# TimeEscaper/distributed_eigenspaces

Hardware: AMD Instinct MI355X
Metric: samples/sec ingested + time-to-eigenspace (d=8192,k=64) at 1/8 GPU; sinθ error (higher is better)
Workload: dtype f32

## Files before the change

__graft_entry__.py:

```python
import os
import sys

ROOT = os.path.dirname(os.path.abspath(__file__))
if ROOT not in sys.path:
    sys.path.insert(0, ROOT)


def build() -> None:
    from distributed_eigenspaces_amd import _build
    _build.build_library(force=True)
    _build.build_oja_timeout_lib()
    import distributed_eigenspaces_amd
    from distributed_eigenspaces_amd import _lib
    _lib.lib()


def smoke() -> None:
    import numpy as np
    import torch

    import distributed_eigenspaces_amd as de
    from oracle import ref_cpu

    dev = torch.device("cuda", 0)
    rng = np.random.default_rng(0)
    d, k, m, n_i = 256, 8, 4, 1024
    U, _ = np.linalg.qr(rng.standard_normal((d, k)))
    X = rng.standard_normal((m * n_i, d)) + (rng.standard_normal((m * n_i, k)) * 2.0) @ U.T
    X = X.astype(np.float32)
    xs = torch.from_numpy(X).to(dev)
    bases = []
    for i in range(m):
        S = de.sigma_hat(xs[i * n_i:(i + 1) * n_i])
        bases.append(de.topk_eigh(S, k).V)
    res = de.projavg_topk(de.stack_bases(bases), k, 1.0 / m, q0=bases[0])
    torch.cuda.synchronize()
    _, _, sw, sv = ref_cpu.one_shot(X.astype(np.float64), k, m)
    dist = ref_cpu.projector_distance(res.V.cpu().numpy(), sv)
    ev_err = np.max(np.abs(res.evals.cpu().numpy() - sw) / np.abs(sw))
    assert dist <= 1e-4, f"smoke: ||P - P_ref||_F = {dist:.3e}"
    assert ev_err <= 1e-5, f"smoke: eigenvalue rel err {ev_err:.3e}"
    print(f"smoke ok: ||P-P_ref||_F={dist:.2e} eig_rel={ev_err:.2e}")


if __name__ == "__main__":
    cmd = sys.argv[1] if len(sys.argv) > 1 else "build"
    {"build": build, "smoke": smoke}[cmd]()
```

distributed_eigenspaces_amd/_build.py:

```python
from __future__ import annotations

import os
import shutil
import subprocess
import sys

HERE = os.path.dirname(os.path.abspath(__file__))
CSRC = os.path.join(HERE, "csrc")
LIB = os.path.join(HERE, "libdeig.so")
SOURCES = ["capi.hip", "syrk.hip", "syrk_split.hip", "syrk_u8.hip", "skinny.hip", "rr.hip", "oja.hip",
           "project.hip", "sweep.hip", "shift.hip"]
EXTRA_FLAGS = {"sweep.hip": ["-fno-slp-vectorize"], "syrk_split.hip": ["-fno-slp-vectorize"]}
HEADERS = ["deig_internal.hpp", os.path.join("..", "..", "include", "deig.h")]
OJA_TIMEOUT_LIB = os.path.join(HERE, "libdeig_test_oja_timeout.so")
ARCH = os.environ.get("DEIG_OFFLOAD_ARCH", "gfx950")


def _hipcc() -> str:
    for cand in (os.environ.get("HIPCC"), "/opt/rocm/bin/hipcc", shutil.which("hipcc")):
        if cand and os.path.exists(cand):
            return cand
    raise RuntimeError("hipcc not found (ROCm required to build libdeig.so)")


def _stale() -> bool:
    if not os.path.exists(LIB):
        return True
    t = os.path.getmtime(LIB)
    deps = [os.path.join(CSRC, s) for s in SOURCES + HEADERS]
    return any(os.path.getmtime(p) > t for p in deps)


def build_library(force: bool = False, verbose: bool = True, defines=(), out: str | None = None) -> str:
    lib = out or LIB
    if not force and not defines and lib == LIB and not _stale():
        return LIB
    objs = []
    tmpdir = os.path.join(HERE, "build" if not defines else "build_ab")
    os.makedirs(tmpdir, exist_ok=True)
    hipcc = _hipcc()
    procs = []
    for src in SOURCES:
        obj = os.path.join(tmpdir, src.replace(".hip", ".o"))
        objs.append(obj)
        cmd = [hipcc, f"--offload-arch={ARCH}", "-O3", "-std=c++17", "-fPIC", "-Wall",
               "-Wno-unused-function", "-Wno-inline-asm"] + list(defines) + EXTRA_FLAGS.get(src, []) + \
            ["-c", os.path.join(CSRC, src), "-o", obj]
        procs.append((cmd, subprocess.Popen(cmd, stdout=subprocess.PIPE, stderr=subprocess.STDOUT)))
    for cmd, p in procs:
        out, _ = p.communicate()
        if p.returncode != 0:
            raise RuntimeError("hipcc failed:\n" + " ".join(cmd) + "\n" + out.decode())
        if verbose and out.strip():
            sys.stderr.write(out.decode())
    tmp_lib = lib + ".tmp"
    cmd = [hipcc, f"--offload-arch={ARCH}", "-shared", "-fPIC", "-o", tmp_lib] + objs
    r = subprocess.run(cmd, stdout=subprocess.PIPE, stderr=subprocess.STDOUT)
    if r.returncode != 0:
        raise RuntimeError("link failed:\n" + r.stdout.decode())
    os.replace(tmp_lib, lib)
    if verbose:
        sys.stderr.write(f"built {lib}\n")
    return lib


def build_oja_timeout_lib(verbose: bool = True) -> str:
    tmpdir = os.path.join(HERE, "build")
    hipcc = _hipcc()
    obj = os.path.join(tmpdir, "oja_timeout.o")
    cmd = [hipcc, f"--offload-arch={ARCH}", "-O3", "-std=c++17", "-fPIC", "-Wall", "-Wno-unused-function",
           "-Wno-inline-asm", "-DDEIG_AB_OJA_SPIN_TICKS=0", "-c", os.path.join(CSRC, "oja.hip"), "-o", obj]
    r = subprocess.run(cmd, stdout=subprocess.PIPE, stderr=subprocess.STDOUT)
    if r.returncode != 0:
        raise RuntimeError("hipcc failed:\n" + " ".join(cmd) + "\n" + r.stdout.decode())
    objs = [obj if s == "oja.hip" else os.path.join(tmpdir, s.replace(".hip", ".o")) for s in SOURCES]
    tmp_lib = OJA_TIMEOUT_LIB + ".tmp"
    r = subprocess.run([hipcc, f"--offload-arch={ARCH}", "-shared", "-fPIC", "-o", tmp_lib] + objs,
                       stdout=subprocess.PIPE, stderr=subprocess.STDOUT)
    if r.returncode != 0:
        raise RuntimeError("link failed:\n" + r.stdout.decode())
    os.replace(tmp_lib, OJA_TIMEOUT_LIB)
    if verbose:
        sys.stderr.write(f"built {OJA_TIMEOUT_LIB}\n")
    return OJA_TIMEOUT_LIB


if __name__ == "__main__":
    build_library(force="--force" in sys.argv)
```

distributed_eigenspaces_amd/csrc/syrk_split.hip:

```cpp
#include <cmath>
#include <cstdlib>

#include "deig_internal.hpp"

namespace deig {
namespace {

typedef __bf16 bf16x8 __attribute__((ext_vector_type(8)));
typedef int i32x4 __attribute__((ext_vector_type(4)));
typedef unsigned u32x4 __attribute__((ext_vector_type(4)));
typedef __bf16 bf16x2 __attribute__((ext_vector_type(2)));
typedef float f32x2 __attribute__((ext_vector_type(2)));

__device__ __forceinline__ uint32_t cvt2(float a, float b) {
  return __builtin_bit_cast(uint32_t, __builtin_convertvector(f32x2{a, b}, bf16x2));
}
__device__ __forceinline__ float lo_f(uint32_t p) { return __uint_as_float(p << 16); }
__device__ __forceinline__ float hi_f(uint32_t p) { return __uint_as_float(p & 0xffff0000u); }

constexpr int BT = 256;
constexpr int ROWS_PAD = 32;
constexpr int NTHR = 512;
constexpr int SLICE_B = BT * 16;
constexpr int SLAB = BT * BT;
constexpr int SPLIT_YB = 256;
constexpr int SUPER_H = 8, SUPER_W = 4;
constexpr int BLOCK_B = 8 * SLICE_B;
constexpr size_t DEFAULT_CHUNK_BYTES = size_t(64) << 30;

struct SSched {
  const unsigned char* XP;
  float* S;
  float* part;
  float* accs;
  const int* order;
  int64_t lds, dp;
  int64_t NK;
  int nseg;
  int d, nt, T, G, q, R;
  float alpha;
  int beta;
  int flush_kt;
  int prio;
  unsigned* pace;
  int pace_kt;
  int xm;
  int rpace;
  const float* X;
  int64_t ldx, nrows;
  float* corr;
};

constexpr int kChipPaceEvery = 2;
#ifdef DEIG_AB_SYRK_FLUSH_STAGGER
constexpr int kFlushStaggerDiv = DEIG_AB_SYRK_FLUSH_STAGGER;
#else
constexpr int kFlushStaggerDiv = 16;
#endif

__device__ __noinline__ void xcd_pace(unsigned* ctr, unsigned target) {
  __hip_atomic_fetch_add(ctr, 1u, __ATOMIC_RELAXED, __HIP_MEMORY_SCOPE_AGENT);
  const uint64_t t0 = wall_clock64();
  while (__hip_atomic_load(ctr, __ATOMIC_RELAXED, __HIP_MEMORY_SCOPE_AGENT) < target) {
    if (wall_clock64() - t0 > 2000) break;
    __builtin_amdgcn_s_sleep(1);
  }
}


__device__ __forceinline__ i32x4 make_rsrc(const void* base, uint32_t nrec) {
  const uint64_t a = reinterpret_cast<uint64_t>(base);
  i32x4 r;
  r[0] = (int)(uint32_t)a;
  r[1] = (int)((uint32_t)(a >> 32) & 0xffffu);
  r[2] = (int)nrec;
  r[3] = 0x00020000;
  return r;
}

__device__ __forceinline__ void dma16(i32x4 rsrc, int voff, const void* lds_dst) {
  const unsigned m0v = (unsigned)(uintptr_t)(lds_void*)lds_dst;
  asm volatile("s_mov_b32 m0, %2\n\tbuffer_load_dwordx4 %0, %1, 0 offen lds"
               :
               : "v"(voff), "s"(rsrc), "s"(m0v)
               : "memory", "m0");
}

template <int KT>
struct Geo {
  static constexpr int NSLICE = 4 * KT;
  static constexpr int PANEL_B = NSLICE * SLICE_B;
  static constexpr int BUF_B = 2 * PANEL_B;
  static constexpr int DMA = 4 * KT, DMA_DIAG = 2 * KT;
};

template <int KT>
__device__ __forceinline__ void stage(const SSched& s, int64_t kt, int i0, int j0, bool diag,
                                      unsigned char* buf, int wave, int lane16) {
  using G_ = Geo<KT>;
  const int64_t blk = kt * KT / 2;
  const int s0 = (int)((kt * KT) & 1) * 4;
  const i32x4 rsrc = make_rsrc(s.XP + blk * (int64_t)s.nt * BLOCK_B, (uint32_t)(s.nt * BLOCK_B));
  int l16 = lane16;
  asm volatile("" : "+v"(l16));
  if (!diag) {
#pragma unroll
    for (int u = 0; u < KT; ++u) {
      const int c = wave * KT + u;
      const int pb = c / G_::NSLICE, sl = c % G_::NSLICE;
      const int g = (pb ? j0 : i0) / BT * BLOCK_B + (s0 + sl) * SLICE_B;
      unsigned char* dst = buf + pb * G_::PANEL_B + sl * SLICE_B;
#pragma unroll
      for (int p = 0; p < 4; ++p) dma16(rsrc, l16 + g + p * 1024, dst + p * 1024);
    }
  } else {
#pragma unroll
    for (int u = 0; u < 2 * KT; ++u) {
      const int idx = wave * 2 * KT + u;
      const int sl = idx >> 2, p = idx & 3;
      dma16(rsrc, l16 + i0 / BT * BLOCK_B + (s0 + sl) * SLICE_B + p * 1024,
            buf + sl * SLICE_B + p * 1024);
    }
  }
}

constexpr int OCT_B = 2 * SLICE_B;

__device__ __forceinline__ void stage_x(const SSched& s, int64_t kt, int f0, unsigned char* buf,
                                        int wave, int voff) {
  const int64_t row0 = kt * 32 + 8 * (wave & 3);
  int64_t rv = s.nrows - row0;
  rv = rv < 0 ? 0 : rv > 8 ? 8 : rv;
  const uint32_t ldx4 = (uint32_t)s.ldx * 4u;
  const i32x4 rsrc = make_rsrc(s.X + row0 * s.ldx + f0, (uint32_t)rv * ldx4);
  unsigned char* dst = buf + (wave >> 2) * Geo<2>::PANEL_B + (wave & 3) * OCT_B;
#pragma unroll
  for (int r = 0; r < 8; ++r) dma16(rsrc, voff + (int)(r * ldx4), dst + r * 1024);
}

template <bool SQ>
__device__ __forceinline__ void convert_x(unsigned char* buf, int wave, int lane, int rv, int fv,
                                          float* sq) {
  unsigned char* R = buf + (wave >> 2) * Geo<2>::PANEL_B + (wave & 3) * OCT_B;
  f32x2 v[2][8];
#pragma unroll
  for (int h = 0; h < 2; ++h)
#pragma unroll
    for (int r = 0; r < 8; ++r)
      v[h][r] = *reinterpret_cast<const f32x2*>(R + r * 1024 + h * 512 + 8 * lane);
  if (rv < 8 || fv < 256) {
#pragma unroll
// ... 334 lines not shown
          stage<KT>(s, k0 + t + NST - 1, i0, j0, diag, lds + nxt * BUF_B, wave, lane16);
        unsigned char* bc = lds + cur * BUF_B;
        acc.template mma<KT>(bc, diag ? bc : bc + Geo<KT>::PANEL_B, wi, wj, lane);
      }
      if (++since == s.flush_kt && t + 1 < nkt) {
        flush<MF>(slab, !flushed, acc, wave, lane);
        wait_vm<0>();
        flushed = true;
        since = 0;
      }
      cur = cur + 1 == NST ? 0 : cur + 1;
      nxt = nxt + 1 == NST ? 0 : nxt + 1;
    }
  }
  if (flushed) unflush<MF>(slab, acc, wave, lane);
  if (sqw) {
    float* c = s.corr + (int64_t)(cseg * 4 + wave) * s.dp + i0;
#pragma unroll
    for (int h = 0; h < 2; ++h)
      *reinterpret_cast<f32x2*>(c + 128 * h + 2 * lane) = f32x2{sq[2 * h], sq[2 * h + 1]};
  }

  if (partial) {
#pragma unroll
    for (int q = 0; q < NQUAD; ++q)
      *slab_at(slab, wave, q, lane) = f32x4{acc.at(q, 0), acc.at(q, 1), acc.at(q, 2), acc.at(q, 3)};
    return;
  }
#pragma unroll
  for (int q = 0; q < NQUAD; ++q) {
    const float a[4] = {acc.at(q, 0), acc.at(q, 1), acc.at(q, 2), acc.at(q, 3)};
    store4(s, i0 + 128 * wi + Acc<MF>::qrow(q, lane), j0 + 64 * wj + Acc<MF>::qcol(q, lane), diag, a);
  }
}

#ifdef DEIG_AB_SYRK_VARIANT
#include "ab/syrk_split_superseded.inc"
#endif

struct PaceSeq {
  int n;
  unsigned base, mult;
  unsigned gbase = 0;
  unsigned gmult = 0;
  bool g = false;
};

__device__ __forceinline__ int rem_active(const SSched& s, int L, int u) {
  if (s.xm) {
    const int gx = s.G >> 3, left = s.R * s.xm - u * gx;
    return left < 0 ? 0 : (left < gx ? left : gx);
  }
  const int xcd = blockIdx.x & 7;
  const int nx = (s.G >> 3) + (xcd < (s.G & 7) ? 1 : 0);
  const int left = s.R * s.nseg - u * s.G - (L - (int)(blockIdx.x >> 3));
  return left < 0 ? 0 : (left < nx ? left : nx);
}

__device__ __forceinline__ int rem_rounds(const SSched& s, int L) {
  if (s.xm) {
    const int gx = s.G >> 3, l = L % gx, items = s.R * s.xm;
    return l < items ? (items - 1 - l) / gx + 1 : 0;
  }
  const int items = s.R * s.nseg;
  return L < items ? (items - 1 - L) / s.G + 1 : 0;
}

__device__ __forceinline__ void rem_item(const SSched& s, int L, int u, int& tile, int& slot, int& sg) {
  int r;
  if (s.xm) {
    const int gx = s.G >> 3, x = L / gx, j = L - x * gx + u * gx;
    const int sl = j / s.R;
    r = j - sl * s.R;
    sg = x * s.xm + sl;
  } else {
    const int i = L + u * s.G;
    sg = i / s.R;
    r = i - sg * s.R;
  }
  tile = s.q * s.G + r;
  slot = sg * s.R + r;
}

constexpr int kDwOff = -1, kDwDiag = -2;
constexpr bool dw_skip(int dw, int mb, int nb) { return dw >= 0 && 16 * mb + 15 < dw + 16 * nb; }
constexpr bool dw_row(int dw, int mb) { return !dw_skip(dw, mb, 0); }
constexpr bool dw_col(int dw, int nb) { return !dw_skip(dw, 7, nb); }
constexpr bool dw_idle(int dw) { return !dw_row(dw, 7); }

template <int PRIO, int DW>
__device__ __forceinline__ void segment_h(const SSched& s, unsigned char* lds, int tile, int64_t k0,
                                          int64_t k1, int slot, bool partial, const PaceSeq& pc) {
  constexpr bool idle = dw_idle(DW);
#ifndef DEIG_AB_SYRK_DIAG_B_DMA
  constexpr bool dgb = DW != kDwOff;
#else
  constexpr bool dgb = false;
#endif
  constexpr int BUF_B = Geo<2>::BUF_B;
  constexpr int QB = 8 * 1024;
  constexpr int BOFF = 4 * QB;
  const int lane = threadIdx.x & 63;
  const int wave = __builtin_amdgcn_readfirstlane(threadIdx.x >> 6);
  const int wi = wave >> 2, wj = wave & 3;
  const bool lag = wave >= 4;
  const int tt = __builtin_amdgcn_readfirstlane(s.order[tile]);
  const int ti = tt & 0xffff, tj = tt >> 16;
  const int i0 = ti * BT, j0 = tj * BT;
  const bool diag = (ti == tj);
  Acc<16> acc;
  acc.zero();
  float* slab = partial ? s.part + (int64_t)slot * SLAB : s.accs + (int64_t)blockIdx.x * SLAB;
  bool flushed = false;
  const int64_t nkt = k1 - k0;
  auto bar = [&]() {
    __builtin_amdgcn_sched_barrier(0);
    __builtin_amdgcn_s_barrier();
    __builtin_amdgcn_sched_barrier(0);
    asm volatile("" ::: "memory");
  };
  const int a_off = ti * BLOCK_B + wave * SLICE_B + ((lane >> 5) * 128 + (lane & 31)) * 16;
  const int b_off = tj * BLOCK_B + wave * SLICE_B + lane * 16;
  const uint32_t nrec = (uint32_t)(s.nt * BLOCK_B);
  auto ring_rsrc = [&](int64_t kt) {
    return make_rsrc(s.XP + kt * (int64_t)s.nt * BLOCK_B, nrec);
  };
  auto issue_a = [&](int64_t kt, int q, unsigned char* buf) {
    const i32x4 r = ring_rsrc(kt);
    int o = a_off + q * 512;
    asm volatile("" : "+v"(o));
    dma16(r, o, buf + q * QB + wave * 1024);
  };
  auto issue_b = [&](int64_t kt, unsigned char* buf, int p0, int p1) {
    const i32x4 r = ring_rsrc(kt);
    int o = b_off;
    asm volatile("" : "+v"(o));
#pragma unroll
    for (int p = 0; p < 4; ++p)
      if (p >= p0 && p < p1) dma16(r, o + p * 1024, buf + BOFF + wave * SLICE_B + p * 1024);
  };
  if (nkt > 0) {
    wait_vm<0>();
    __syncthreads();
    if constexpr (!dgb) issue_b(k0, lds, 0, 4);
#pragma unroll
    for (int q = 0; q < 4; ++q) issue_a(k0, q, lds);
    if (nkt > 1) {
      if constexpr (!dgb) issue_b(k0 + 1, lds + BUF_B, 0, 2);
      issue_a(k0 + 1, 0, lds + BUF_B);
      issue_a(k0 + 1, 1, lds + BUF_B);
      wait_vm<dgb ? 2 : 4>();
    } else {
      wait_vm<0>();
    }
    asm volatile("s_waitcnt lgkmcnt(0)" ::: "memory");
    bar();
    if (lag) bar();
    const int c = lane & 15, g4 = lane >> 4;
    const int xcd = blockIdx.x & 7;
    int since = kFlushStaggerDiv > 0 ? xcd * (s.flush_kt / kFlushStaggerDiv) : 0;
    int since_pace = 0, pace_left = pc.n;
    unsigned pace_t = pc.base;
    int gcount = 0;
    unsigned gtarget = pc.gbase;
    bf16x8 bhi[4], blo[4];
    bf16x8 ahi[4], alo[4];
    for (int64_t t = 0; t < nkt; ++t) {
      unsigned char* cur = lds + (t & 1) * BUF_B;
      unsigned char* nxt = lds + ((t + 1) & 1) * BUF_B;
      const bool has1 = t + 1 < nkt, has2 = t + 2 < nkt;
      const unsigned char* pa = cur + ((g4 * 2) * 64 + 32 * wi + c) * 16;
      const unsigned char* pb = cur + BOFF + ((g4 * 2) * BT + 64 * wj + c) * 16;
      const unsigned char* pbd = cur + (2 * (wj & 1)) * QB + (2 * g4) * 1024 + (32 * (wj >> 1) + c) * 16;
#pragma unroll
      for (int h = 0; h < 2; ++h) {
        if (h == 0) {
          if (pace_left > 0 && ++since_pace == s.pace_kt) {
            since_pace = 0;
            --pace_left;
            pace_t += pc.mult;
            if (threadIdx.x == 0) xcd_pace(s.pace + 32 * xcd, pace_t);
            if (pc.g && ++gcount == kChipPaceEvery) {
              gcount = 0;
              gtarget += pc.gmult;
              if (threadIdx.x == 0) xcd_pace(s.pace + 32 * 8, gtarget);
            }
          }
          if (since == s.flush_kt) {
            if constexpr (!idle) flush<16>(slab, !flushed, acc, wave, lane);
            wait_vm<0>();
            flushed = true;
            since = 0;
          }
          ++since;
          if (has1) {
            if constexpr (!dgb) issue_b(k0 + t + 1, nxt, 2, 4);
            issue_a(k0 + t + 1, 2, nxt);
            issue_a(k0 + t + 1, 3, nxt);
          }
#pragma unroll
          for (int nb = 0; nb < 4; ++nb) {
            if (dw_col(DW, nb)) {
              if constexpr (dgb) {
                const unsigned char* pq = pbd + (nb >> 1) * QB + (16 * (nb & 1)) * 16;
                bhi[nb] = *reinterpret_cast<const bf16x8*>(pq);
                blo[nb] = *reinterpret_cast<const bf16x8*>(pq + 1024);
              } else {
                bhi[nb] = *reinterpret_cast<const bf16x8*>(pb + (16 * nb) * 16);
                blo[nb] = *reinterpret_cast<const bf16x8*>(pb + (BT + 16 * nb) * 16);
              }
            }
          }
        } else if (has2) {
          if constexpr (!dgb) issue_b(k0 + t + 2, cur, 0, 2);
          issue_a(k0 + t + 2, 0, cur);
          issue_a(k0 + t + 2, 1, cur);
        }
#pragma unroll
        for (int m = 0; m < 4; ++m) {
          const int q = 2 * h + (m >> 1), mm = m & 1;
          if (dw_row(DW, 4 * h + m)) {
            ahi[m] = *reinterpret_cast<const bf16x8*>(pa + q * QB + (16 * mm) * 16);
            alo[m] = *reinterpret_cast<const bf16x8*>(pa + q * QB + (64 + 16 * mm) * 16);
          }
        }
        if constexpr (dgb) {
          if (h == 0) {
            if (has1) wait_vm<4>(); else wait_vm<0>();
          } else {
            if (has2) wait_vm<2>(); else wait_vm<0>();
          }
        } else if (h == 0) {
          if (has1) wait_vm<8>(); else wait_vm<0>();
        } else {
          if (has2) wait_vm<6>(); else if (has1) wait_vm<2>(); else wait_vm<0>();
        }
        asm volatile("s_waitcnt lgkmcnt(0)" ::: "memory");
        bar();
        if (PRIO) __builtin_amdgcn_s_setprio(1);
#pragma unroll
        for (int m = 0; m < 4; ++m) {
          const int mb = 4 * h + m;
#pragma unroll
          for (int nb = 0; nb < 4; ++nb)
            if (!dw_skip(DW, mb, nb))
              acc.a[mb][nb] = __builtin_amdgcn_mfma_f32_16x16x32_bf16(ahi[m], bhi[nb], acc.a[mb][nb], 0, 0, 0);
#pragma unroll
          for (int nb = 0; nb < 4; ++nb)
            if (!dw_skip(DW, mb, nb))
              acc.a[mb][nb] = __builtin_amdgcn_mfma_f32_16x16x32_bf16(ahi[m], blo[nb], acc.a[mb][nb], 0, 0, 0);
#pragma unroll
          for (int nb = 0; nb < 4; ++nb)
            if (!dw_skip(DW, mb, nb))
              acc.a[mb][nb] = __builtin_amdgcn_mfma_f32_16x16x32_bf16(alo[m], bhi[nb], acc.a[mb][nb], 0, 0, 0);
        }
        if (PRIO) __builtin_amdgcn_s_setprio(0);
        bar();
      }
    }
    if (!lag) bar();
  }
  if (flushed && !idle) unflush<16>(slab, acc, wave, lane);
  if (partial) {
#pragma unroll
    for (int q = 0; q < NQUAD; ++q)
      *slab_at(slab, wave, q, lane) = f32x4{acc.at(q, 0), acc.at(q, 1), acc.at(q, 2), acc.at(q, 3)};
    return;
  }
  if constexpr (idle) return;
#pragma unroll
  for (int q = 0; q < NQUAD; ++q) {
    const float a[4] = {acc.at(q, 0), acc.at(q, 1), acc.at(q, 2), acc.at(q, 3)};
    store4(s, i0 + 128 * wi + Acc<16>::qrow(q, lane), j0 + 64 * wj + Acc<16>::qcol(q, lane), diag, a);
  }
}

template <int PRIO>
__global__ __launch_bounds__(NTHR) void syrks_h_kernel(SSched s) {
  __shared__ __attribute__((aligned(16))) unsigned char lds[2 * Geo<2>::BUF_B];
  const int L = xcd_logical(blockIdx.x, s.G);
  const int nwork = s.q + rem_rounds(s, L);
  const int xcd = blockIdx.x & 7;
  const unsigned nx = (unsigned)((s.G >> 3) + (xcd < (s.G & 7) ? 1 : 0));
  const unsigned P = s.pace_kt > 0 ? (unsigned)(s.NK / s.pace_kt) : 0u;
  const int Pm = (s.pace_kt > 0 && s.rpace && s.nseg > 0) ? (int)(s.NK / s.nseg / s.pace_kt) : 0;
  unsigned rbase = (unsigned)s.q * P * nx;
  for (int w = 0; w < nwork; ++w) {
    int tile, slot = 0, sg = 0;
    int64_t k0 = 0, k1 = s.NK;
    const bool partial = w >= s.q;
    PaceSeq pc{0, 0u, 0u};
    if (!partial) {
      tile = w * s.G + L;
      pc = PaceSeq{(int)P, (unsigned)w * P * nx, nx};
      pc.g = true;
      pc.gbase = (unsigned)w * (P / kChipPaceEvery) * (unsigned)s.G;
      pc.gmult = (unsigned)s.G;
    } else {
      rem_item(s, L, w - s.q, tile, slot, sg);
      k0 = __builtin_amdgcn_readfirstlane((int)(s.NK * sg / s.nseg));
      k1 = __builtin_amdgcn_readfirstlane((int)(s.NK * (sg + 1) / s.nseg));
      if (Pm > 0) {
        unsigned before = 0;
        for (int u = 0; u < w - s.q; ++u) before += (unsigned)rem_active(s, L, u);
        pc = PaceSeq{Pm, rbase + before * (unsigned)Pm, (unsigned)rem_active(s, L, w - s.q)};
#ifndef DEIG_AB_SYRK_NO_REM_CHIP
        if (!s.xm) {
          const int items = s.R * s.nseg;
          unsigned gb = (unsigned)s.q * (P / kChipPaceEvery) * (unsigned)s.G;
          for (int u = 0; u < w - s.q; ++u)
            gb += (unsigned)min(s.G, items - u * s.G) * (unsigned)(Pm / kChipPaceEvery);
          pc.g = true;
          pc.gbase = gb;
          pc.gmult = (unsigned)min(s.G, items - (w - s.q) * s.G);
        }
#endif
      }
    }
    const int tt = __builtin_amdgcn_readfirstlane(s.order[tile]);
    const int wv = __builtin_amdgcn_readfirstlane(threadIdx.x >> 6);
    const bool dg = (tt & 0xffff) == (tt >> 16);
#ifndef DEIG_AB_SYRK_NO_DIAG_IDLE
    const int dw = 64 * (wv & 3) - 128 * (wv >> 2);
    if (dg && dw == 0)
      segment_h<PRIO, 0>(s, lds, tile, k0, k1, slot, partial, pc);
    else if (dg && dw == 64)
      segment_h<PRIO, 64>(s, lds, tile, k0, k1, slot, partial, pc);
    else if (dg && dw >= 128)
      segment_h<PRIO, 128>(s, lds, tile, k0, k1, slot, partial, pc);
    else if (dg)
      segment_h<PRIO, kDwDiag>(s, lds, tile, k0, k1, slot, partial, pc);
    else
#endif
      segment_h<PRIO, kDwOff>(s, lds, tile, k0, k1, slot, partial, pc);
  }
}

template <int MF, int KT, int NST, bool FX>
__global__ __launch_bounds__(NTHR) void syrks_kernel(SSched s) {
  static_assert(NST * Geo<KT>::BUF_B <= 160 * 1024, "LDS ring exceeds 160 KiB");
  __shared__ __attribute__((aligned(16))) unsigned char lds[NST * Geo<KT>::BUF_B];
  const int b = blockIdx.x;
  const int L = xcd_logical(b, s.G);
  const int items = s.R * s.nseg;
  const int nwork = s.q + (L < items ? (items - 1 - L) / s.G + 1 : 0);
  for (int w = 0; w < nwork; ++w) {
    int tile, slot = 0, cseg = 0;
    int64_t k0 = 0, k1 = s.NK;
    const bool partial = w >= s.q;
    if (!partial) {
      tile = w * s.G + L;
    } else {
      const int i = L + (w - s.q) * s.G;
      const int sg = i / s.R, r = i - sg * s.R;
      tile = s.q * s.G + r;
      slot = i;
      cseg = sg;
      k0 = __builtin_amdgcn_readfirstlane((int)(s.NK * sg / s.nseg));
      k1 = __builtin_amdgcn_readfirstlane((int)(s.NK * (sg + 1) / s.nseg));
    }
    const int pace_j = (!partial && s.pace_kt > 0) ? (int)(w * (s.NK / s.pace_kt)) : -1;
    if constexpr (FX) {
      const int tt = __builtin_amdgcn_readfirstlane(s.order[tile]);
      if ((tt & 0xffff) == (tt >> 16) && (threadIdx.x >> 6) < 4)
        segment<MF, KT, NST, true, true>(s, lds, tile, k0, k1, slot, partial, pace_j, cseg);
      else
        segment<MF, KT, NST, true, false>(s, lds, tile, k0, k1, slot, partial, pace_j, cseg);
    } else {
      segment<MF, KT, NST, false, false>(s, lds, tile, k0, k1, slot, partial, pace_j, cseg);
    }
  }
}

template <int MF>
__global__ __launch_bounds__(256) void syrks_reduce_kernel(SSched s) {
  const int r = blockIdx.x;
  const int f = blockIdx.y * 256 + threadIdx.x;
  const int lane = f & 63, q = (f >> 6) & (NQUAD - 1), wave = f >> 11;
  const int wi = wave >> 2, wj = wave & 3;
  const int tt = s.order[s.q * s.G + r];
  const int ti = tt & 0xffff, tj = tt >> 16;
  const bool diag = (ti == tj);
  f32x4 sum = {0.f, 0.f, 0.f, 0.f};
  for (int sg = 0; sg < s.nseg; ++sg)
    sum += *reinterpret_cast<const f32x4*>(s.part + (int64_t)(sg * s.R + r) * SLAB + (int64_t)f * 4);
  const float a[4] = {sum[0], sum[1], sum[2], sum[3]};
  store4(s, ti * BT + 128 * wi + Acc<MF>::qrow(q, lane), tj * BT + 64 * wj + Acc<MF>::qcol(q, lane),
         diag, a);
}

__device__ __forceinline__ uint32_t bf16_rne(float x) {
  const uint32_t u = __float_as_uint(x);
  return (u + 0x7fffu + ((u >> 16) & 1u)) >> 16;
}

__global__ __launch_bounds__(256) void split_kernel(const float* __restrict__ X, int64_t n,
                                                    int64_t ldx, int d, int64_t dp, int64_t noct,
// ... 50 lines not shown
  const int i = blockIdx.x * 64 + t;
  float c = 0.f;
  if (i < d) {
#pragma unroll 8
    for (int y = sl; y < yb; y += 4) c += corr[(int64_t)y * dp + i];
  }
  part[sl][t] = c;
  __syncthreads();
  if (sl == 0 && i < d) S[(int64_t)i * lds + i] += alpha * (((part[0][t] + part[1][t]) + part[2][t]) + part[3][t]);
}

__global__ __launch_bounds__(256) void tile_order_kernel(int nt, int* order) {
  const int nsc = (nt + SUPER_W - 1) / SUPER_W;
  const int u = blockIdx.x * 256 + threadIdx.x;
  const int R0 = (u / nsc) * SUPER_H, C0 = (u % nsc) * SUPER_W;
  if (R0 >= nt) return;
  const int rmax = R0 + SUPER_H < nt ? R0 + SUPER_H : nt;
  if (C0 >= rmax) return;
  int idx = R0 * (R0 + 1) / 2;
  for (int c = 0; c < C0; c += SUPER_W)
    for (int ti = R0; ti < rmax; ++ti) {
      const int hi = c + SUPER_W < ti + 1 ? c + SUPER_W : ti + 1;
      idx += hi > c ? hi - c : 0;
    }
  for (int ti = R0; ti < rmax; ++ti)
    for (int tj = C0; tj < C0 + SUPER_W && tj <= ti; ++tj) order[idx++] = ti | (tj << 16);
}

int remainder_segments(int64_t R, int G) {
  if (R <= 0) return 0;
  double best = 1e30;
  for (int k = 1; k <= 64; ++k) best = fmin(best, (double)cdiv(R * k, G) / k);
  for (int k = 1; k <= 64; ++k)
    if ((double)cdiv(R * k, G) / k <= best * 1.02) return k;
  return 1;
}

__global__ __launch_bounds__(256) void tile_order_compact_kernel(int nt, int* order) {
  const int m = nt / 8;
  const int u = blockIdx.x * 256 + threadIdx.x;
  if (u >= m * m) return;
  int a = (int)sqrtf((float)u);
  while (a * a > u) --a;
  while ((a + 1) * (a + 1) <= u) ++a;
  const int item = u - a * a;
  int* grp = order + 32 * u;
  if (item == 0) {
    int i = 0;
    for (int ti = 8 * a; ti < 8 * a + 8; ++ti)
      for (int tj = 8 * a; tj <= ti; ++tj) {
        const int v = ti | (tj << 16);
        if (i < 32) grp[i] = v;
        else order[32 * m * m + 4 * a + (i - 32)] = v;
        ++i;
      }
  } else {
    const int b = (item - 1) >> 1, h = (item - 1) & 1;
    int i = 0;
    for (int ti = 8 * a; ti < 8 * a + 8; ++ti)
      for (int tj = 8 * b + 4 * h; tj < 8 * b + 4 * h + 4; ++tj) grp[i++] = ti | (tj << 16);
  }
}

#ifdef DEIG_AB_SYRK_REM
constexpr int kSyrkRem = DEIG_AB_SYRK_REM;
#else
constexpr int kSyrkRem = 1;
#endif
int syrk_variant(int64_t d);

int xcd_segments(int64_t R, int gx) {
  double best = 1e30;
  for (int k = 1; k <= 8; ++k) best = fmin(best, (double)cdiv(R * k, gx) / (8 * k));
  for (int k = 1; k <= 8; ++k)
    if ((double)cdiv(R * k, gx) / (8 * k) <= best * 1.02) return k;
  return 1;
}

struct Layout {
  int64_t dp, nt, T, G, q, R, nseg, xm, yb_max, chunk_rows;
  size_t off_order, off_pace, off_accs, off_part, off_corr, off_xp, total;
};

Layout make_layout(int64_t n, int64_t d, int G, int64_t chunk_rows) {
  Layout L;
  L.dp = cdiv(d, BT) * BT;
  L.nt = L.dp / BT;
  L.T = L.nt * (L.nt + 1) / 2;
  L.G = G;
  L.q = L.T / G;
  L.R = L.T % G;
  L.nseg = remainder_segments(L.R, G);
  L.xm = 0;
  if ((kSyrkRem & 2) && syrk_variant(d) % 100000 >= 30000 && G % 8 == 0 && L.R > 0) {
    L.xm = xcd_segments(L.R, G / 8);
    L.nseg = 8 * L.xm;
  }
  L.yb_max = SPLIT_YB;
  L.chunk_rows = chunk_rows;
  size_t off = 0;
  L.off_order = off;
  off = align_up(off + sizeof(int) * L.T, 256);
  L.off_pace = off;
  off += 16 * 128;
  L.off_accs = off;
  off += sizeof(float) * (size_t)G * SLAB;
  L.off_part = off;
  off += sizeof(float) * (size_t)(L.R * L.nseg) * SLAB;
  L.off_corr = off;
  off = align_up(off + sizeof(float) * (size_t)L.yb_max * L.dp, 256);
  L.off_xp = off;
  off += (size_t)chunk_rows * L.dp * 4;
  L.total = off;
  (void)n;
  return L;
}

int64_t default_chunk_rows(int64_t n, int64_t d) {
  const int64_t dp = cdiv(d, BT) * BT;
  const int64_t n32 = cdiv(n, ROWS_PAD) * ROWS_PAD;
  int64_t cap = (int64_t)(DEFAULT_CHUNK_BYTES / (size_t)(dp * 4)) / ROWS_PAD * ROWS_PAD;
  if (cap < ROWS_PAD) cap = ROWS_PAD;
  return n32 < cap ? n32 : cap;
}

constexpr int64_t kFusedMaxD = 2048;
#ifdef DEIG_AB_SYRK_VARIANT
constexpr int kSyrkLarge = DEIG_AB_SYRK_VARIANT;
#else
constexpr int kSyrkLarge = 30000;
#endif
int syrk_variant(int64_t d) {
#ifdef DEIG_AB_SYRK_VARIANT
  (void)d;
  return DEIG_AB_SYRK_VARIANT;
#else
  return d <= kFusedMaxD ? 163 : kSyrkLarge;
#endif
}

template <int V>
void launch_split_pass_kernel(int G, hipStream_t stream, const SSched& s) {
  if constexpr (V % 100000 >= 30000) {
    hipLaunchKernelGGL((syrks_h_kernel<(V / 10) % 10>), dim3(G), dim3(NTHR), 0, stream, s);
  }
#ifdef DEIG_AB_SYRK_VARIANT
  else if constexpr (V % 100000 >= 20000) {
    hipLaunchKernelGGL((syrks_q_kernel<(V / 10) % 10, V / 100000, (V / 100) % 10>), dim3(G), dim3(NTHR), 0,
                       stream, s);
  } else if constexpr (V >= 10000) {
    hipLaunchKernelGGL((syrks_st_kernel<(V / 1000) % 10, (V / 100) % 10, (V / 10) % 10, V / 100000>), dim3(G),
                       dim3(NTHR), 0, stream, s);
  } else if constexpr (V == 13 || V == 14 || V == 15) {
    hipLaunchKernelGGL((syrks_kernel<32, 1, V - 10, false>), dim3(G), dim3(NTHR), 0, stream, s);
  } else if constexpr (V == 22) {
    hipLaunchKernelGGL((syrks_kernel<32, 2, 2, false>), dim3(G), dim3(NTHR), 0, stream, s);
  } else {
    hipLaunchKernelGGL((syrks_kernel<16, 2, 2, false>), dim3(G), dim3(NTHR), 0, stream, s);
  }
#else
  else {
    static_assert(V % 100000 >= 30000, "the shipped library has only the half-refill ring");
  }
#endif
}

}

int syrk_cus() {
#ifdef DEIG_AB_SYRK_G
  return DEIG_AB_SYRK_G;
#else
  return num_cus();
#endif
}

size_t syrk_split_workspace_bytes(int64_t n, int64_t d) {
  if (n < 1 || d < 1) return 0;
  if (syrk_variant(d) == 163) return make_layout(n, d, syrk_cus(), 0).total;
  return make_layout(n, d, syrk_cus(), default_chunk_rows(n, d)).total;
}

int syrk_split_launch(const float* X, int64_t n, int64_t d, int64_t ldx, float alpha, float* S,
                      int64_t lds, void* ws, size_t ws_bytes, hipStream_t stream, bool accumulate) {
  DEIG_REQUIRE(n >= 1, "syrk: n must be >= 1 (got %lld)", (long long)n);
  DEIG_REQUIRE(d >= 1 && d % 4 == 0, "syrk: d must be a positive multiple of 4 (got %lld)",
               (long long)d);
  DEIG_REQUIRE(d <= (1 << 16) - BT, "syrk: d too large (%lld)", (long long)d);
  DEIG_REQUIRE(ldx >= d && ldx % 4 == 0, "syrk: ldx must be >= d and a multiple of 4");
  DEIG_REQUIRE(lds >= d && lds % 4 == 0, "syrk: lds must be >= d and a multiple of 4");
  DEIG_REQUIRE(X && S && aligned16(X) && aligned16(S), "syrk: X and S must be 16-byte aligned");
  const int G = syrk_cus();
  const int variant = syrk_variant(d);
  const bool fused = variant == 163;
  Layout L0 = make_layout(n, d, G, 0);
  const size_t ws_min = L0.total + (fused ? 0 : (size_t)ROWS_PAD * L0.dp * 4);
  if (!ws || ws_bytes < ws_min)
    return fail(DEIG_EWORKSPACE, "syrk: workspace %zu bytes < minimum %zu", ws_bytes, ws_min);
  int64_t chunk = (int64_t)((ws_bytes - L0.total) / (size_t)(L0.dp * 4)) / ROWS_PAD * ROWS_PAD;
  const int64_t n32 = cdiv(n, ROWS_PAD) * ROWS_PAD;
  if (chunk > n32) chunk = n32;
  const Layout L = make_layout(n, d, G, fused ? 0 : chunk);
  char* base = static_cast<char*>(ws);

  SSched s;
  s.S = S;
  s.lds = lds;
  s.dp = L.dp;
  s.d = (int)d;
  s.nt = (int)L.nt;
  s.T = (int)L.T;
  s.G = G;
  s.q = (int)L.q;
  s.R = (int)L.R;
  s.alpha = alpha;
  s.order = reinterpret_cast<const int*>(base + L.off_order);
  s.accs = reinterpret_cast<float*>(base + L.off_accs);
  s.part = reinterpret_cast<float*>(base + L.off_part);
  s.XP = reinterpret_cast<const unsigned char*>(base + L.off_xp);
  float* corr = reinterpret_cast<float*>(base + L.off_corr);
  unsigned char* xp = reinterpret_cast<unsigned char*>(base + L.off_xp);

#ifdef DEIG_AB_SYRK_FLUSH_ROWS
  int64_t flush_rows = DEIG_AB_SYRK_FLUSH_ROWS;
#else
  int64_t flush_rows = 4096;
  while (flush_rows < 16384 && (flush_rows * 2) * (flush_rows * 2) <= 128 * n) flush_rows *= 2;
#endif
  s.prio = 0;
  s.pace = reinterpret_cast<unsigned*>(base + L.off_pace);
#ifdef DEIG_AB_SYRK_PACE
  s.pace_kt = DEIG_AB_SYRK_PACE;
#else
  s.pace_kt = 64;
#endif
  s.xm = (int)L.xm;
  s.rpace = kSyrkRem & 1;
#ifndef DEIG_AB_SYRK_SUPER_ORDER
  if (G == 256 && s.nt % 8 == 0)
    hipLaunchKernelGGL(tile_order_compact_kernel, dim3((unsigned)cdiv((s.nt / 8) * (s.nt / 8), 256)), dim3(256), 0,
                       stream, s.nt, reinterpret_cast<int*>(base + L.off_order));
  else
#endif
    hipLaunchKernelGGL(tile_order_kernel,
                       dim3((unsigned)cdiv(cdiv(s.nt, SUPER_H) * cdiv(s.nt, SUPER_W), 256)), dim3(256), 0, stream,
                       s.nt, reinterpret_cast<int*>(base + L.off_order));
  DEIG_HIP_CHECK(hipGetLastError());
  s.X = X;
  s.ldx = ldx;
  s.nrows = n;
  s.corr = corr;
  if (fused) {
    DEIG_REQUIRE(ldx <= (int64_t(1) << 25), "syrk: ldx > 2^25 is not supported for d <= 2048");
    const int64_t yb = 4 * (L.nseg > 1 ? L.nseg : 1);
    DEIG_REQUIRE(yb <= L.yb_max, "syrk: %lld lo^2 partial rows exceed the workspace's %lld",
                 (long long)yb, (long long)L.yb_max);
    DEIG_HIP_CHECK(hipMemsetAsync(corr, 0, sizeof(float) * (size_t)(yb * L.dp), stream));
    s.NK = cdiv(n, ROWS_PAD);
    s.nseg = (int)L.nseg;
    s.beta = accumulate ? 1 : 0;
    s.flush_kt = (int)(flush_rows / ROWS_PAD);
    if (s.flush_kt < 1) s.flush_kt = 1;
    if (s.pace_kt > 0) DEIG_HIP_CHECK(hipMemsetAsync(s.pace, 0, 9 * 128, stream));
    hipLaunchKernelGGL((syrks_kernel<16, 2, 2, true>), dim3(G), dim3(NTHR), 0, stream, s);
    DEIG_HIP_CHECK(hipGetLastError());
    if (s.R > 0) {
      hipLaunchKernelGGL(syrks_reduce_kernel<16>, dim3(s.R, SLAB / 4 / 256), dim3(256), 0, stream, s);
      DEIG_HIP_CHECK(hipGetLastError());
    }
    hipLaunchKernelGGL(diag_corr_kernel, dim3((unsigned)cdiv(d, 64)), dim3(256), 0, stream, corr,
                       (int)yb, L.dp, (int)d, alpha, S, lds);
    DEIG_HIP_CHECK(hipGetLastError());
    return DEIG_OK;
  }
  for (int64_t r0 = 0, c = 0; r0 < n; r0 += chunk, ++c) {
    const int64_t rows = (n - r0) < chunk ? (n - r0) : chunk;
    const int64_t nk32 = cdiv(rows, ROWS_PAD);
    const int64_t noct = nk32 * (ROWS_PAD / 8);
    const int kt_steps = (variant >= 13 && variant <= 15) ? 1 : 2;
    const int64_t nk = nk32 * (ROWS_PAD / 16) / kt_steps;
    int64_t yb = cdiv(noct, 4);
    if (yb > L.yb_max) yb = L.yb_max;
    hipLaunchKernelGGL(split_kernel, dim3((unsigned)(L.dp / 256), (unsigned)yb), dim3(256), 0,
                       stream, X + r0 * ldx, rows, ldx, (int)d, L.dp, noct, xp, corr);
    DEIG_HIP_CHECK(hipGetLastError());
    s.NK = nk;
    s.nseg = (int)L.nseg;
    s.beta = (c > 0 || accumulate) ? 1 : 0;
    s.flush_kt = (int)(flush_rows / (16 * kt_steps));
    const bool mf16 = variant >= 100;
    if (s.pace_kt > 0) DEIG_HIP_CHECK(hipMemsetAsync(s.pace, 0, 9 * 128, stream));
    if (variant != 163) launch_split_pass_kernel<kSyrkLarge == 163 ? 162 : kSyrkLarge>(G, stream, s);
    DEIG_HIP_CHECK(hipGetLastError());
    if (s.R > 0) {
      if (mf16)
        hipLaunchKernelGGL(syrks_reduce_kernel<16>, dim3(s.R, SLAB / 4 / 256), dim3(256), 0, stream, s);
      else
        hipLaunchKernelGGL(syrks_reduce_kernel<32>, dim3(s.R, SLAB / 4 / 256), dim3(256), 0, stream, s);
      DEIG_HIP_CHECK(hipGetLastError());
    }
    hipLaunchKernelGGL(diag_corr_kernel, dim3((unsigned)cdiv(d, 64)), dim3(256), 0, stream, corr,
                       (int)yb, L.dp, (int)d, alpha, S, lds);
    DEIG_HIP_CHECK(hipGetLastError());
  }
  return DEIG_OK;
}

}
```

Baseline: 7.259 million.

## Replace flat chip-wide pacing barrier with hierarchical per-XCD leader pacing in SYRK

Chip-level pacing in the split SYRK kernel becomes hierarchical. Each XCD counts arrivals on its own line, the last arriving block publishes an epoch to a per-XCD chip slot and waits for all active XCDs, then releases its siblings through a per-XCD release line. This replaces every block spinning on a single chip-wide counter, cutting atomic contention on one cache line at the cost of more pace lines, a larger memset and more complex wait logic. Optional timestamp instrumentation and A/B build variants (unpaced, G=250) are added behind compile-time flags.

```diff
diff --git a/__graft_entry__.py b/__graft_entry__.py
--- a/__graft_entry__.py
+++ b/__graft_entry__.py
@@ -10,6 +10,7 @@
     from distributed_eigenspaces_amd import _build
     _build.build_library(force=True)
     _build.build_oja_timeout_lib()
+    _build.build_syrk_pacing_libs()
     import distributed_eigenspaces_amd
     from distributed_eigenspaces_amd import _lib
     _lib.lib()
diff --git a/distributed_eigenspaces_amd/_build.py b/distributed_eigenspaces_amd/_build.py
--- a/distributed_eigenspaces_amd/_build.py
+++ b/distributed_eigenspaces_amd/_build.py
@@ -13,6 +13,12 @@
 EXTRA_FLAGS = {"sweep.hip": ["-fno-slp-vectorize"], "syrk_split.hip": ["-fno-slp-vectorize"]}
 HEADERS = ["deig_internal.hpp", os.path.join("..", "..", "include", "deig.h")]
 OJA_TIMEOUT_LIB = os.path.join(HERE, "libdeig_test_oja_timeout.so")
+SYRK_PACING_LIBS = {
+    "unpaced": (os.path.join(HERE, "libdeig_test_syrk_unpaced.so"), ["-DDEIG_AB_SYRK_PACE=0"]),
+    "g250": (os.path.join(HERE, "libdeig_test_syrk_g250.so"), ["-DDEIG_AB_SYRK_G=250"]),
+    "g250_unpaced": (os.path.join(HERE, "libdeig_test_syrk_g250_unpaced.so"),
+                     ["-DDEIG_AB_SYRK_G=250", "-DDEIG_AB_SYRK_PACE=0"]),
+}
 ARCH = os.environ.get("DEIG_OFFLOAD_ARCH", "gfx950")
 
 
@@ -85,5 +91,30 @@
     return OJA_TIMEOUT_LIB
 
 
+def build_syrk_pacing_libs(verbose: bool = True) -> dict:
+    tmpdir = os.path.join(HERE, "build")
+    hipcc = _hipcc()
+    procs = []
+    for name, (lib, defs) in SYRK_PACING_LIBS.items():
+        obj = os.path.join(tmpdir, f"syrk_split_{name}.o")
+        cmd = [hipcc, f"--offload-arch={ARCH}", "-O3", "-std=c++17", "-fPIC", "-Wall", "-Wno-unused-function",
+               "-Wno-inline-asm"] + defs + EXTRA_FLAGS["syrk_split.hip"] + \
+            ["-c", os.path.join(CSRC, "syrk_split.hip"), "-o", obj]
+        procs.append((lib, obj, cmd, subprocess.Popen(cmd, stdout=subprocess.PIPE, stderr=subprocess.STDOUT)))
+    for lib, obj, cmd, p in procs:
+        out, _ = p.communicate()
+        if p.returncode != 0:
+            raise RuntimeError("hipcc failed:\n" + " ".join(cmd) + "\n" + out.decode())
+        objs = [obj if s == "syrk_split.hip" else os.path.join(tmpdir, s.replace(".hip", ".o")) for s in SOURCES]
+        r = subprocess.run([hipcc, f"--offload-arch={ARCH}", "-shared", "-fPIC", "-o", lib + ".tmp"] + objs,
+                           stdout=subprocess.PIPE, stderr=subprocess.STDOUT)
+        if r.returncode != 0:
+            raise RuntimeError("link failed:\n" + r.stdout.decode())
+        os.replace(lib + ".tmp", lib)
+        if verbose:
+            sys.stderr.write(f"built {lib}\n")
+    return {name: lib for name, (lib, _) in SYRK_PACING_LIBS.items()}
+
+
 if __name__ == "__main__":
     build_library(force="--force" in sys.argv)
diff --git a/distributed_eigenspaces_amd/csrc/syrk_split.hip b/distributed_eigenspaces_amd/csrc/syrk_split.hip
--- a/distributed_eigenspaces_amd/csrc/syrk_split.hip
+++ b/distributed_eigenspaces_amd/csrc/syrk_split.hip
@@ -51,7 +51,60 @@
   float* corr;
 };
 
+#ifdef DEIG_AB_SYRK_CHIP_EVERY
+constexpr int kChipPaceEvery = DEIG_AB_SYRK_CHIP_EVERY;
+#else
 constexpr int kChipPaceEvery = 2;
+#endif
+#ifdef DEIG_AB_SYRK_CHIP_FLAT
+constexpr bool kChipHier = false;
+#else
+constexpr bool kChipHier = true;
+#endif
+constexpr int kPaceChipLine = 8, kPaceRelLine = 9, kPaceLines = 17;
+constexpr uint64_t kPaceSpinTicks = 2000;
+
+#ifdef DEIG_AB_SYRK_STAMPS
+constexpr int kStampWords = 8;
+__device__ __forceinline__ uint64_t stamp() {
+  uint64_t t;
+  __builtin_amdgcn_sched_barrier(0);
+  asm volatile("s_memtime %0\n\ts_waitcnt lgkmcnt(0)" : "=s"(t)::"memory");
+  __builtin_amdgcn_sched_barrier(0);
+  return t;
+}
+__device__ __forceinline__ unsigned long long* stamp_slot(unsigned* pace, int i) {
+  return reinterpret_cast<unsigned long long*>(pace + 32 * kPaceLines) + (size_t)blockIdx.x * kStampWords + i;
+}
+#define DEIG_STAMP_TIMEOUT(pace) atomicAdd(stamp_slot(pace, 5), 1ull)
+#define DEIG_STAMP_VARS() uint64_t st_t0 = 0, st_seg = wave == 0 ? stamp() : 0, st_sum[8] = {}
+#define DEIG_STAMP_BEGIN() \
+  do {                     \
+    if (wave == 0) st_t0 = stamp(); \
+  } while (0)
+#define DEIG_STAMP_END(slot, cnt)              \
+  do {                                         \
+    if (wave == 0) {                           \
+      st_sum[slot] += stamp() - st_t0;         \
+      if ((cnt) >= 0) st_sum[(cnt) & 7] += 1;  \
+    }                                          \
+  } while (0)
+#define DEIG_STAMP_FLUSH()                                        \
+  do {                                                            \
+    if (wave == 0) {                                              \
+      st_sum[4] = stamp() - st_seg;                               \
+      if (lane == 0)                                              \
+        for (int i = 0; i < 8; ++i)                               \
+          if (i != 5) atomicAdd(stamp_slot(s.pace, i), (unsigned long long)st_sum[i]); \
+    }                                                             \
+  } while (0)
+#else
+#define DEIG_STAMP_TIMEOUT(pace) ((void)0)
+#define DEIG_STAMP_VARS() ((void)0)
+#define DEIG_STAMP_BEGIN() ((void)0)
+#define DEIG_STAMP_END(slot, cnt) ((void)0)
+#define DEIG_STAMP_FLUSH() ((void)0)
+#endif
 #ifdef DEIG_AB_SYRK_FLUSH_STAGGER
 constexpr int kFlushStaggerDiv = DEIG_AB_SYRK_FLUSH_STAGGER;
 #else
@@ -62,11 +115,13 @@
   __hip_atomic_fetch_add(ctr, 1u, __ATOMIC_RELAXED, __HIP_MEMORY_SCOPE_AGENT);
   const uint64_t t0 = wall_clock64();
   while (__hip_atomic_load(ctr, __ATOMIC_RELAXED, __HIP_MEMORY_SCOPE_AGENT) < target) {
-    if (wall_clock64() - t0 > 2000) break;
+    if (wall_clock64() - t0 > kPaceSpinTicks) {
+      DEIG_STAMP_TIMEOUT(ctr - 32 * (blockIdx.x & 7));
+      break;
+    }
     __builtin_amdgcn_s_sleep(1);
   }
 }
-
 
 __device__ __forceinline__ i32x4 make_rsrc(const void* base, uint32_t nrec) {
   const uint64_t a = reinterpret_cast<uint64_t>(base);
@@ -567,6 +622,63 @@
   slot = sg * s.R + r;
 }
 
+__device__ __noinline__ void pace_point(unsigned* pace_v, unsigned xtarget_v, unsigned epoch_nax_v) {
+  const unsigned pace_lo = (unsigned)__builtin_amdgcn_readfirstlane((int)(unsigned)(uintptr_t)pace_v);
+  const unsigned pace_hi = (unsigned)__builtin_amdgcn_readfirstlane((int)(unsigned)((uintptr_t)pace_v >> 32));
+  unsigned* pace = reinterpret_cast<unsigned*>((uint64_t)pace_hi << 32 | (uint64_t)pace_lo);
+  const unsigned xtarget = __builtin_amdgcn_readfirstlane(xtarget_v);
+  const unsigned epoch_nax = __builtin_amdgcn_readfirstlane(epoch_nax_v);
+  const unsigned epoch = epoch_nax >> 4;
+  const unsigned nax = epoch_nax & 15u;
+  const int xcd = blockIdx.x & 7;
+  const unsigned lane = __builtin_amdgcn_mbcnt_hi(~0u, __builtin_amdgcn_mbcnt_lo(~0u, 0u));
+  unsigned old = 0;
+  if (lane == 0) old = __hip_atomic_fetch_add(pace + 32 * xcd, 1u, __ATOMIC_RELAXED, __HIP_MEMORY_SCOPE_AGENT);
+  old = __builtin_amdgcn_readfirstlane(old);
+  unsigned* rel = pace + 32 * (kPaceRelLine + xcd);
+  const uint64_t t0 = wall_clock64();
+  if (epoch_nax == 0) {
+    for (;;) {
+      unsigned c = 0;
+      if (lane == 0) c = __hip_atomic_load(pace + 32 * xcd, __ATOMIC_RELAXED, __HIP_MEMORY_SCOPE_AGENT);
+      if (__builtin_amdgcn_readfirstlane(c) >= xtarget) break;
+      if (wall_clock64() - t0 > kPaceSpinTicks) {
+        if (lane == 0) DEIG_STAMP_TIMEOUT(pace);
+        break;
+      }
+      __builtin_amdgcn_s_sleep(1);
+    }
+  } else if (old + 1u == xtarget) {
+    unsigned* chip = pace + 32 * kPaceChipLine;
+    if (lane == 0) __hip_atomic_fetch_max(chip + xcd, epoch, __ATOMIC_RELAXED, __HIP_MEMORY_SCOPE_AGENT);
+    for (;;) {
+      bool ok = true;
+      if (lane < nax) ok = __hip_atomic_load(chip + lane, __ATOMIC_RELAXED, __HIP_MEMORY_SCOPE_AGENT) >= epoch;
+      if (__all(ok)) break;
+      if (wall_clock64() - t0 > kPaceSpinTicks) {
+        if (lane == 0) DEIG_STAMP_TIMEOUT(pace);
+        break;
+      }
+      __builtin_amdgcn_s_sleep(1);
+    }
+    if (lane == 0) __hip_atomic_fetch_max(rel, epoch, __ATOMIC_RELAXED, __HIP_MEMORY_SCOPE_AGENT);
+  } else {
+    for (;;) {
+      unsigned r = 0;
+      if (lane == 0) r = __hip_atomic_load(rel, __ATOMIC_RELAXED, __HIP_MEMORY_SCOPE_AGENT);
+      if (__builtin_amdgcn_readfirstlane(r) >= epoch) break;
+      if (wall_clock64() - t0 > kPaceSpinTicks) {
+        if (lane == 0) DEIG_STAMP_TIMEOUT(pace);
+        break;
+      }
+      __builtin_amdgcn_s_sleep(1);
+    }
+  }
+  asm volatile("s_waitcnt vmcnt(0)" ::: "memory");
+}
+
+
+
 constexpr int kDwOff = -1, kDwDiag = -2;
 constexpr bool dw_skip(int dw, int mb, int nb) { return dw >= 0 && 16 * mb + 15 < dw + 16 * nb; }
 constexpr bool dw_row(int dw, int mb) { return !dw_skip(dw, mb, 0); }
@@ -589,6 +701,8 @@
   const int wave = __builtin_amdgcn_readfirstlane(threadIdx.x >> 6);
   const int wi = wave >> 2, wj = wave & 3;
   const bool lag = wave >= 4;
+  DEIG_STAMP_VARS();
+  DEIG_STAMP_BEGIN();
   const int tt = __builtin_amdgcn_readfirstlane(s.order[tile]);
   const int ti = tt & 0xffff, tj = tt >> 16;
   const int i0 = ti * BT, j0 = tj * BT;
@@ -650,6 +764,7 @@
     unsigned gtarget = pc.gbase;
     bf16x8 bhi[4], blo[4];
     bf16x8 ahi[4], alo[4];
+    DEIG_STAMP_END(3, -1);
     for (int64_t t = 0; t < nkt; ++t) {
       unsigned char* cur = lds + (t & 1) * BUF_B;
       unsigned char* nxt = lds + ((t + 1) & 1) * BUF_B;
@@ -664,16 +779,31 @@
             since_pace = 0;
             --pace_left;
             pace_t += pc.mult;
-            if (threadIdx.x == 0) xcd_pace(s.pace + 32 * xcd, pace_t);
-            if (pc.g && ++gcount == kChipPaceEvery) {
-              gcount = 0;
-              gtarget += pc.gmult;
-              if (threadIdx.x == 0) xcd_pace(s.pace + 32 * 8, gtarget);
+            if (kChipHier) {
+              const unsigned j = (unsigned)(pc.n - pace_left);
+              const bool chip = pc.g && j % kChipPaceEvery == 0;
+              DEIG_STAMP_BEGIN();
+              if (wave == 0) pace_point(s.pace, pace_t, chip ? pc.gbase + ((j / kChipPaceEvery) << 4) : 0u);
+              DEIG_STAMP_END(chip ? 1 : 0, chip ? 7 : 6);
+            } else {
+              const bool chip = pc.g && ++gcount == kChipPaceEvery;
+              if (chip) gcount = 0;
+              DEIG_STAMP_BEGIN();
+              if (threadIdx.x == 0) xcd_pace(s.pace + 32 * xcd, pace_t);
+              DEIG_STAMP_END(0, 6);
+              if (chip) {
+                gtarget += pc.gmult;
+                DEIG_STAMP_BEGIN();
+                if (threadIdx.x == 0) xcd_pace(s.pace + 32 * kPaceChipLine, gtarget);
+                DEIG_STAMP_END(1, 7);
+              }
             }
           }
           if (since == s.flush_kt) {
+            DEIG_STAMP_BEGIN();
             if constexpr (!idle) flush<16>(slab, !flushed, acc, wave, lane);
             wait_vm<0>();
+            DEIG_STAMP_END(2, -1);
             flushed = true;
             since = 0;
           }
@@ -743,6 +873,7 @@
         bar();
       }
     }
+    DEIG_STAMP_BEGIN();
     if (!lag) bar();
   }
   if (flushed && !idle) unflush<16>(slab, acc, wave, lane);
@@ -750,14 +881,22 @@
 #pragma unroll
     for (int q = 0; q < NQUAD; ++q)
       *slab_at(slab, wave, q, lane) = f32x4{acc.at(q, 0), acc.at(q, 1), acc.at(q, 2), acc.at(q, 3)};
+    DEIG_STAMP_END(3, -1);
+    DEIG_STAMP_FLUSH();
     return;
   }
-  if constexpr (idle) return;
+  if constexpr (idle) {
+    DEIG_STAMP_END(3, -1);
+    DEIG_STAMP_FLUSH();
+    return;
+  }
 #pragma unroll
   for (int q = 0; q < NQUAD; ++q) {
     const float a[4] = {acc.at(q, 0), acc.at(q, 1), acc.at(q, 2), acc.at(q, 3)};
     store4(s, i0 + 128 * wi + Acc<16>::qrow(q, lane), j0 + 64 * wj + Acc<16>::qcol(q, lane), diag, a);
   }
+  DEIG_STAMP_END(3, -1);
+  DEIG_STAMP_FLUSH();
 }
 
 template <int PRIO>
@@ -779,8 +918,12 @@
       tile = w * s.G + L;
       pc = PaceSeq{(int)P, (unsigned)w * P * nx, nx};
       pc.g = true;
-      pc.gbase = (unsigned)w * (P / kChipPaceEvery) * (unsigned)s.G;
-      pc.gmult = (unsigned)s.G;
+      if (kChipHier) {
+        pc.gbase = ((unsigned)w * (P / kChipPaceEvery)) << 4 | (unsigned)min(s.G, 8);
+      } else {
+        pc.gbase = (unsigned)w * (P / kChipPaceEvery) * (unsigned)s.G;
+        pc.gmult = (unsigned)s.G;
+      }
     } else {
       rem_item(s, L, w - s.q, tile, slot, sg);
       k0 = __builtin_amdgcn_readfirstlane((int)(s.NK * sg / s.nseg));
@@ -792,12 +935,20 @@
 #ifndef DEIG_AB_SYRK_NO_REM_CHIP
         if (!s.xm) {
           const int items = s.R * s.nseg;
-          unsigned gb = (unsigned)s.q * (P / kChipPaceEvery) * (unsigned)s.G;
-          for (int u = 0; u < w - s.q; ++u)
-            gb += (unsigned)min(s.G, items - u * s.G) * (unsigned)(Pm / kChipPaceEvery);
+          const int cnt = min(s.G, items - (w - s.q) * s.G);
           pc.g = true;
-          pc.gbase = gb;
-          pc.gmult = (unsigned)min(s.G, items - (w - s.q) * s.G);
+          if (kChipHier) {
+            unsigned nax = 0;
+            for (int x = 0; x < 8; ++x) nax += xcd_logical(x, s.G) < cnt ? 1u : 0u;
+            pc.gbase = ((unsigned)s.q * (P / kChipPaceEvery) + (unsigned)(w - s.q) * (unsigned)(Pm / kChipPaceEvery))
+                           << 4 | nax;
+          } else {
+            unsigned gb = (unsigned)s.q * (P / kChipPaceEvery) * (unsigned)s.G;
+            for (int u = 0; u < w - s.q; ++u)
+              gb += (unsigned)min(s.G, items - u * s.G) * (unsigned)(Pm / kChipPaceEvery);
+            pc.gbase = gb;
+            pc.gmult = (unsigned)cnt;
+          }
         }
 #endif
       }
@@ -1014,6 +1165,15 @@
   size_t off_order, off_pace, off_accs, off_part, off_corr, off_xp, total;
 };
 
+size_t pace_bytes(int G) {
+#ifdef DEIG_AB_SYRK_STAMPS
+  return align_up((size_t)kPaceLines * 128 + sizeof(uint64_t) * kStampWords * (size_t)G, 256);
+#else
+  (void)G;
+  return align_up((size_t)kPaceLines * 128, 256);
+#endif
+}
+
 Layout make_layout(int64_t n, int64_t d, int G, int64_t chunk_rows) {
   Layout L;
   L.dp = cdiv(d, BT) * BT;
@@ -1034,7 +1194,7 @@
   L.off_order = off;
   off = align_up(off + sizeof(int) * L.T, 256);
   L.off_pace = off;
-  off += 16 * 128;
+  off += pace_bytes(G);
   L.off_accs = off;
   off += sizeof(float) * (size_t)G * SLAB;
   L.off_part = off;
@@ -1106,6 +1266,13 @@
   return num_cus();
 #endif
 }
+
+#ifdef DEIG_AB_SYRK_STAMPS
+extern "C" __attribute__((visibility("default"))) size_t deig_ab_syrk_stamp_offset(int64_t n, int64_t d, int* G) {
+  *G = syrk_cus();
+  return make_layout(n, d, *G, 0).off_pace + (size_t)kPaceLines * 128;
+}
+#endif
 
 size_t syrk_split_workspace_bytes(int64_t n, int64_t d) {
   if (n < 1 || d < 1) return 0;
@@ -1193,7 +1360,7 @@
     s.beta = accumulate ? 1 : 0;
     s.flush_kt = (int)(flush_rows / ROWS_PAD);
     if (s.flush_kt < 1) s.flush_kt = 1;
-    if (s.pace_kt > 0) DEIG_HIP_CHECK(hipMemsetAsync(s.pace, 0, 9 * 128, stream));
+    if (s.pace_kt > 0) DEIG_HIP_CHECK(hipMemsetAsync(s.pace, 0, pace_bytes(G), stream));
     hipLaunchKernelGGL((syrks_kernel<16, 2, 2, true>), dim3(G), dim3(NTHR), 0, stream, s);
     DEIG_HIP_CHECK(hipGetLastError());
     if (s.R > 0) {
@@ -1221,7 +1388,7 @@
     s.beta = (c > 0 || accumulate) ? 1 : 0;
     s.flush_kt = (int)(flush_rows / (16 * kt_steps));
     const bool mf16 = variant >= 100;
-    if (s.pace_kt > 0) DEIG_HIP_CHECK(hipMemsetAsync(s.pace, 0, 9 * 128, stream));
+    if (s.pace_kt > 0) DEIG_HIP_CHECK(hipMemsetAsync(s.pace, 0, pace_bytes(G), stream));
     if (variant != 163) launch_split_pass_kernel<kSyrkLarge == 163 ? 162 : kSyrkLarge>(G, stream, s);
     DEIG_HIP_CHECK(hipGetLastError());
     if (s.R > 0) {
```

Result: no change. 7.314 million (median of 6 runs) (+0.8%).
